# cure-lab/MagicDrive

Measured on AMD Instinct MI355X. Metric: 6-view scenes/sec at 224x400, 50-step DDIM, higher is better.
Workload: dtype bf16; 1 GPU; configs[1]: 6-view 224x400, text-only conditioning (camera_param=None -> CFG off), 50-step DDIM, bf16; scenes_per_gpu=64, ddim_steps=50, scheduler=ddim, parallelism=scene-sharded x1, hipgraph=True, streams=2, output_type=latent

## Files before the change

magicdrive_amd/csrc/gemm_route.h:

```cpp
#pragma once
#include <cstddef>
#include <cstdio>

#if defined(__HIPCC__) || defined(__HIP__)
#define MDX_ROUTE_HD __host__ __device__ __forceinline__
#else
#define MDX_ROUTE_HD inline
#endif

namespace mdx_route {

constexpr int R_EINVAL = -1, R_EUNSUPPORTED = -3;
constexpr int XL_SLOTS = 12;

struct RouteIn {
    int M, N, K, batch, splitk, epi;
    bool c_f32, conv;
    int Hi, Wi, Cin, Ho, Wo, kh, kw, sh, sw, ph, pw;
    bool cimajor, up2;
    int upB;
    long lda, ldw, ldc, ldr, sC;
    int rows_per_b, col_split;
    long ws_bytes;
    bool has_ws, bias, temb, R, Vt, Wq, ln_csum, ln_scratch, ln_stats, rowstat;
    int ln_stats_parts, rowstat_parts;
    bool ln;
    bool wide;
    bool r_al16, wq_al16, bias_al16;
};

struct RouteOpts {
    int GEMM_WS, GEMM_XL, XL_K320, XL_MIN_TILES, XL_BN, XL_GEGLU320, GEMM_SMALL_TILES, GEMM_BM256, GEMM_BM, GEMM_BN, GEMM_BK, GEMM_FLATTEN,
        LN_FUSE, LN_STATS, GEMM_TIMING;
};

enum Main { MAIN_WS, MAIN_XL, MAIN_GENERIC };

struct Route {
    int err;
    const char* msg;
    int arg;
    Main main;
    int bn;
    int BM, BN, BK, splitk, kchunk;
    bool normalise_first;
    bool rowstat_after;
    bool keep_rowstat, keep_ln, keep_ln_stats;
    bool timing;
};

struct UpAxis { int cnt, first, pad, par; };
MDX_ROUTE_HD UpAxis up_axis(int c, int n_in, int n_out) {
    const int crop = n_out != 2 * n_in;
    UpAxis a;
    a.cnt = c == 2 ? 1 : n_in - crop;
    a.first = c == 2 ? n_in - 1 : 0;
    a.pad = c == 1 ? 0 : 1;
    a.par = c == 1 ? 1 : 0;
    return a;
}
MDX_ROUTE_HD int up_mtiles(int upB, int Hi, int Wi, int Ho, int Wo) {
    const int ny = 2 + (Ho != 2 * Hi), nx = 2 + (Wo != 2 * Wi);
    int mt = 0;
    for (int yc = 0; yc < ny; ++yc)
        for (int xc = 0; xc < nx; ++xc) mt += (int)(((long)upB * up_axis(yc, Hi, Ho).cnt * up_axis(xc, Wi, Wo).cnt + 255) / 256);
    return mt;
}

inline bool xl_supported(const RouteIn& p, int bn) {
    const bool conv = p.conv;
    if (p.batch > 1 || p.splitk > 1 || p.c_f32 || (p.N % 4) || (p.K % 64) || p.Vt) return false;
    if (p.col_split && (conv || p.bias || p.temb || p.R || p.epi || (p.sC & 1) || (p.ldc & 1) || p.col_split < 16)) return false;
    if (bn != 256 && bn != 160 && bn != 320) return false;
    if (p.epi == 1 && (bn != 256 || (p.N % 64))) return false;
    if (p.epi == 2) return false;
    if (conv && p.up2) {
        if (bn == 160 || p.kh != 2 || p.kw != 2 || (p.Cin % 64) || p.R || p.temb || p.epi || p.col_split) return false;
        if (p.upB < 1 || p.Hi < 1 || p.Wi < 1 || (p.Ho != 2 * p.Hi && p.Ho != 2 * p.Hi - 1) || (p.Wo != 2 * p.Wi && p.Wo != 2 * p.Wi - 1)) return false;
        if ((long)p.Hi * p.Wi + 256 >= (1L << 24) || (long)p.upB * p.Hi * p.Wi >= 0x7fffff00L) return false;
        const long span = ((long)(256 / p.Wi + 3) * p.Wi + 256L + 2 * p.Wi) * p.lda * 2;
        if (span >= 0x40000000L) return false;
        if ((p.Ho != 2 * p.Hi || p.Wo != 2 * p.Wi) && ((long)p.upB * p.Hi * p.Wi + p.Wi + 2) * p.lda * 2 >= 0x7fff0000L) return false;
    } else if (conv) {
        if (p.kh != 3 || p.kw != 3 || p.ph != 1 || p.pw != 1 || (p.Cin % 64) || !p.cimajor) return false;
        const long span = ((long)(256 / p.Wo + 3) * p.sh * p.Wi + 256L * p.sw + 3 * p.Wi) * p.lda * 2;
        if (span >= 0x40000000L) return false;
    } else if ((long)256 * p.lda * 2 >= 0x40000000L) return false;
    if ((long)bn * p.ldw * 2 >= 0x40000000L) return false;
    if (p.temb && p.epi != 1) {
        const int rows = p.rows_per_b > 0 ? p.rows_per_b : 1;
        if (256 / rows + 2 > XL_SLOTS) return false;
    }
    return true;
}

inline bool ws_supported(const RouteIn& p) {
    return p.K == 320 && p.batch <= 1 && p.splitk <= 1 && !p.c_f32 && !p.temb && (p.epi == 0 || p.epi == 1) && (p.N % 4) == 0 &&
           (p.epi != 1 || (p.N % 64) == 0);
}
inline bool ws_fits_window(const RouteIn& p) { return (long)p.M * p.lda * 2 < 0x7FFF0000L; }
inline bool ws_fuses_layernorm(const RouteIn& p) {
    if (!p.ln_csum || (p.ln_stats && p.ln_stats_parts > 4)) return false;
    return p.epi == 0 || (p.epi == 1 && p.ln_stats);
}
inline bool ws_emits_rowstat(const RouteIn& p) {
    return p.rowstat && p.epi == 0 && !p.Vt && p.wide && !p.c_f32 && !p.ln && (p.N + 127) / 128 <= p.rowstat_parts;
}
inline bool xd_supported(const RouteIn& q) {
    if (!q.Wq || q.batch > 1 || q.splitk > 1 || q.c_f32 || q.Vt || q.col_split || q.temb || q.rowstat || q.ln) return false;
    if (q.epi != 0 && q.epi != 1) return false;
    if (q.epi == 1 && (q.R || (q.N % 64))) return false;
    if ((q.K % 128) || q.K < 640 || (q.N % 16) || !q.wide) return false;
    if (q.R && ((q.ldr % 8) || !q.r_al16)) return false;
    if (!q.wq_al16 || (q.bias && !q.bias_al16)) return false;
    if ((long)256 * q.lda * 2 >= 0x40000000L || (long)256 * q.ldc * 2 >= 0x40000000L || (long)256 * q.ldr * 2 >= 0x40000000L) return false;
    if ((long)16 * (q.K >> 5) * 1024 >= 0x40000000L) return false;
    return true;
}

struct XlWidth { int bn; unsigned bit; double a, b; };
constexpr unsigned W320 = 1, W256 = 2, W160 = 4, W_ALL = 7;
constexpr XlWidth kXlWidths[3] = {{320, W320, 23.7, 1.896}, {256, W256, 13.4, 1.565}, {160, W160, 16.6, 1.116}};
inline unsigned xl_width_bit(int bn) { return bn == 320 ? W320 : bn == 256 ? W256 : bn == 160 ? W160 : 0u; }

inline int xl_pick_width(const RouteIn& p, long mtiles, long min_tiles, unsigned widths) {
    int pick = 0;
    double best = 1e300;
    for (const XlWidth& w : kXlWidths) {
        if (!(widths & w.bit) || !xl_supported(p, w.bn)) continue;
        const long t = mtiles * ((p.N + w.bn - 1) / w.bn);
        if (t < min_tiles) continue;
        const double c = (double)((t + 255) / 256) * (w.a + w.b * (p.K / 64.0));
        if (c < best) { best = c; pick = w.bn; }
    }
    return pick;
}

inline Route route_fail(Route r, int code, const char* msg, int arg = 0) { r.err = code; r.msg = msg; r.arg = arg; return r; }
inline Route route_xl(Route r, int bn) { r.main = MAIN_XL; r.bn = bn; return r; }

inline Route gemm_route_flat(const RouteIn& p, const RouteOpts& o) {
    Route r = {};
    const int bn = o.GEMM_XL > 0 ? xl_pick_width(p, (p.M + 255) / 256, 128, W_ALL) : 0;
    return bn ? route_xl(r, bn) : route_fail(r, R_EUNSUPPORTED, nullptr);
}

inline Route gemm_route(RouteIn p, const RouteOpts& o) {
    Route r = {};
    r.main = MAIN_GENERIC;
    const bool conv = p.conv, geglu = p.epi == 1;
    if (!o.LN_STATS) { p.rowstat = false; p.rowstat_parts = 0; p.ln_stats = false; p.ln_stats_parts = 0; }
    r.keep_rowstat = p.rowstat; r.keep_ln = p.ln; r.keep_ln_stats = p.ln_stats;
    if (p.up2) {
        if (!conv) return route_fail(r, R_EINVAL, "upsample2x: conv only");
        int bn = xl_pick_width(p, up_mtiles(p.upB, p.Hi, p.Wi, p.Ho, p.Wo), 0, W320 | W256);
        if ((o.XL_BN == 320 || o.XL_BN == 256) && xl_supported(p, o.XL_BN)) bn = o.XL_BN;
        if (!bn) return route_fail(r, R_EINVAL, "mdx_conv2d: upsample2x needs Cin %% 64 == 0, Ho in {2 Hi, 2 Hi - 1}, Wo in {2 Wi, 2 Wi - 1}, bias-only epilogue, no split-K; with a cropped axis B * Hi * Wi * ldx * 2 < 2^31");
        return route_xl(r, bn);
    }
    if (geglu && (p.N % 64) != 0) return route_fail(r, R_EINVAL, "GEGLU needs packed N %% 64 == 0 (N=%d)", p.N);
    const long mt256 = (p.M + 255) / 256;
    const bool geglu_xl = o.XL_GEGLU320 && o.GEMM_XL == 1 && !conv && geglu && p.K == 320 && p.splitk <= 1 && o.GEMM_WS < 2 &&
                          xl_supported(p, 256) && mt256 * ((p.N + 255) / 256) >= 1024;
    const bool ws_first = !conv && o.GEMM_WS > 0 && p.splitk <= 1 && ws_supported(p) && ws_fits_window(p) && (o.GEMM_WS >= 2 || p.M >= 8192);
    const bool ws_taken = !geglu_xl && ws_first && !(o.XL_K320 && o.GEMM_XL > 0);
    if (p.rowstat) {
        if (conv || p.batch > 1 || p.epi != 0 || p.c_f32 || p.Vt || p.rowstat_parts < 1) return route_fail(r, R_EINVAL, "rowstat_out: plain 2-D GEMM with 16-bit C only");
        if (!(ws_taken && ws_emits_rowstat(p) && o.LN_FUSE)) {
            r.rowstat_after = true; r.keep_rowstat = false;
            p.rowstat = false; p.rowstat_parts = 0;
        }
    }
    if (p.ln) {
        if (conv || p.batch > 1) return route_fail(r, R_EINVAL, "fused LayerNorm: plain 2-D GEMM only");
        if (!(ws_taken && ws_fuses_layernorm(p) && o.LN_FUSE)) {
            if (!p.ln_scratch) return route_fail(r, R_EINVAL, "fused LayerNorm: this shape is not normalised in-kernel and no ln_scratch was given");
            r.normalise_first = true; r.keep_ln = r.keep_ln_stats = false;
            p.ln = false; p.ln_csum = false; p.ln_stats = false; p.ln_stats_parts = 0;
        }
    }
    const unsigned widths = o.XL_BN ? xl_width_bit(o.XL_BN) : W_ALL;
    if (o.GEMM_XL >= 2 && p.splitk <= 1 && p.batch <= 1 && !(p.K == 320 && !conv && !o.XL_K320)) {
        if (const int bn = xl_pick_width(p, mt256, 0, widths)) return route_xl(r, bn);
    }
    if (geglu_xl) return route_xl(r, 256);
    if (ws_taken) { r.main = MAIN_WS; return r; }
    int BM, BN = 128;
    if (!geglu && (p.N <= 64 || (p.N % 128 != 0 && p.N <= 192))) BN = 64;
    BM = p.M >= 2048 ? 128 : 64;
    if (o.GEMM_SMALL_TILES && p.batch <= 1) {
        const long t64 = (long)((p.M + 63) / 64) * ((p.N + 63) / 64);
        if (geglu) {
            BM = p.M >= 512 ? 128 : 64;
        } else if (!conv) {
            if (t64 <= 1408) BM = BN = 64;
        } else if (t64 * (long)((p.K + 63) / 64) <= 40000) {
            BM = BN = 64;
        } else if (BN == 128) {
            BM = 128;
        }
    }
    if (o.GEMM_BM256 && BN == 128 && p.M >= o.GEMM_BM256) BM = 256;
    if (o.GEMM_BM == 64 || o.GEMM_BM == 128) BM = o.GEMM_BM;
    if ((o.GEMM_BN == 64 && !geglu) || o.GEMM_BN == 128) BN = o.GEMM_BN;
    const long tiles = (long)((p.M + BM - 1) / BM) * ((p.N + BN - 1) / BN) * (p.batch > 1 ? p.batch : 1);
    int splitk = 1;
    if (p.splitk > 0) {
        splitk = p.splitk;
    } else if (p.batch <= 1 && p.has_ws && tiles < 384 && p.K >= 1024 && (p.N % 4) == 0) {
        const long want = (768 + tiles - 1) / tiles;
        const long maxs = p.K / 512;
        splitk = (int)(want < maxs ? (want < 32 ? want : 32) : (maxs < 32 ? maxs : 32));
        if (splitk < 1) splitk = 1;
    }
    if (p.batch > 1) splitk = 1;
    if (splitk > 1) {
        const long per = (long)p.M * p.N * (long)sizeof(float);
        const long fit = per > 0 ? p.ws_bytes / per : 0;
        if (fit < splitk) splitk = fit < 1 ? 1 : (int)fit;
    }
    const int kchunk = ((p.K + splitk - 1) / splitk + 63) / 64 * 64;
    splitk = (p.K + kchunk - 1) / kchunk;
    if (splitk > 1 && !p.has_ws) return route_fail(r, R_EINVAL, "split-K needs a workspace");
    p.splitk = splitk;
    if (splitk == 1 && o.GEMM_XL > 0) {
        if (const int bn = xl_pick_width(p, mt256, o.GEMM_XL >= 2 ? 0 : o.XL_MIN_TILES, widths)) return route_xl(r, bn);
    }
    if (ws_first) { r.main = MAIN_WS; return r; }
    r.BM = BM; r.BN = BN; r.BK = o.GEMM_BK == 32 ? 32 : 64; r.splitk = splitk; r.kchunk = kchunk;
    r.timing = o.GEMM_TIMING && p.has_ws && splitk == 1;
    return r;
}

inline void tag_generic(char* s, size_t n, int BM, int BN, int BK, bool conv) {
    snprintf(s, n, "gemm_conv_kernel<%d,%d,%d,%d,%d,%s>", BM, BN, BK, BM == 256 ? 4 : 2, 2, conv ? "conv" : "gemm");
}
inline void tag_xl(char* s, size_t n, int bn, bool conv, bool up2) {
    snprintf(s, n, "gemm_xl_kernel<256x%d,%s>", bn, conv ? (up2 ? "conv,up2x" : "conv") : "gemm");
}
inline void tag_xlp(char* s, size_t n, bool geglu, bool has_r) {
    snprintf(s, n, "gemm_xlp_kernel<256x256,%s%s>", geglu ? "geglu" : "gemm", has_r ? "+res" : "");
}
inline const char* tag_ws(bool geglu, bool vt, int ln, bool rs) {
    return geglu ? (ln ? "gemm_ws_kernel<geglu,lns>" : "gemm_ws_kernel<geglu>")
                 : ln == 2 ? (vt ? "gemm_ws_kernel<vT,lns>" : "gemm_ws_kernel<plain,lns>")
                 : ln == 1 ? (vt ? "gemm_ws_kernel<vT,ln>" : "gemm_ws_kernel<plain,ln>")
                           : (vt ? "gemm_ws_kernel<vT>" : rs ? "gemm_ws_kernel<plain,rs>" : "gemm_ws_kernel<plain>");
}
inline void route_tag(const Route& r, const RouteIn& p, char* s, size_t n) {
    if (r.main == MAIN_XL) tag_xl(s, n, r.bn, p.conv, p.up2);
    else if (r.main == MAIN_GENERIC) tag_generic(s, n, r.BM, r.BN, r.BK, p.conv);
    else snprintf(s, n, "%s", tag_ws(p.epi == 1, false, !r.keep_ln ? 0 : r.keep_ln_stats ? 2 : 1, r.keep_rowstat));
}

}
```

magicdrive_amd/csrc/gemm_ws.hip:

```cpp
#include "common.h"
#include "launch.h"
#include "options.h"
#include "gemm_params.h"

namespace mdx {

constexpr unsigned WS_OOB = 0xFFFFFF00u;
constexpr unsigned WS_RECORDS = 0x80000000u;

template <int N>
__device__ __forceinline__ void ws_wait_vmcnt() { asm volatile("s_waitcnt vmcnt(%0)" ::"n"(N) : "memory"); }
typedef __attribute__((ext_vector_type(4))) unsigned ws_rsrc_t;
__device__ __forceinline__ void ws_glds(const ws_rsrc_t rs, unsigned lds_addr, unsigned voff) {
    unsigned keep;
    lds_addr = __builtin_amdgcn_readfirstlane(lds_addr);
    asm volatile(
        "s_mov_b32 %0, m0\n\t"
        "s_mov_b32 m0, %1\n\t"
        "s_nop 0\n\t"
        "buffer_load_dwordx4 %2, %3, 0 offen lds\n\t"
        "s_mov_b32 m0, %0"
        : "=&s"(keep)
        : "s"(lds_addr), "v"(voff), "s"(rs)
        : "memory");
}
__device__ __forceinline__ void ws_lds_barrier() {
    asm volatile("s_waitcnt lgkmcnt(0)" ::: "memory");
    __builtin_amdgcn_s_barrier();
    asm volatile("" ::: "memory");
}

template <bool GEGLU, int ST, bool VT, int LN, bool RS>
__global__ __launch_bounds__(256, 2) void gemm_ws_kernel(GCParams p) {
    static_assert(!(GEGLU && LN == 1), "in-kernel LayerNorm statistics: plain and V^T epilogues only");
    static_assert(!(RS && (GEGLU || VT)), "row statistics: plain store phase only");

    constexpr int BM = 128, BN = 128, BK = 64, KS = 20, NSLAB = 5;
    constexpr int BNO = GEGLU ? BN / 2 : BN;
    constexpr int CSTR = BNO + 8;
    constexpr int ROWS_PASS = GEGLU ? 128 : 64;
    constexpr int CSTR_T = ROWS_PASS + 8;
    constexpr int STAGE = BM * BK * 2;
    constexpr int PPW = 4;
    extern __shared__ __attribute__((aligned(16))) unsigned char smem[];
    bf16_t* Cs = (bf16_t*)(smem + ST * STAGE);
    float2* Ls = (float2*)(smem + ST * STAGE + 128 * (64 + 8) * 2);
    float* Lc = (float*)(Ls + 128);
    float* Lb = Lc + 128;

    const int tid = threadIdx.x, lane = tid & 63;
    const int wave = __builtin_amdgcn_readfirstlane(tid >> 6);
    const int frow = lane & 31, half = lane >> 5;
    const int xcd = blockIdx.x & 7, kq = blockIdx.x >> 3;
    const int tn = kq % p.nt;
    const int walker = (kq / p.nt) * 8 + xcd;
    const int nwalk = p.swz;
    const int n0 = tn * BN;
    const int mt = p.mt;
    const int ntiles = walker < mt ? (mt - walker + nwalk - 1) / nwalk : 0;
    if (ntiles == 0) return;

    int wrow, ocol;
    if (GEGLU) {
        const int grp = wave >> 1, hv = wave & 1;
        wrow = n0 + grp * 64 + (frow < 16 ? 16 * hv + frow : 32 + 16 * hv + (frow - 16));
        ocol = grp * 32 + 16 * hv;
    } else {
        wrow = n0 + 32 * wave + frow;
        ocol = 32 * wave;
    }
    Frag8 wf[KS];
    {
        const bf16_t* wp = p.W + (long)min(wrow, p.N - 1) * p.ldw + half * 8;
        const unsigned keep = wrow < p.N ? 0xffffffffu : 0u;
#pragma unroll
        for (int ks = 0; ks < KS; ++ks) wf[ks].u = *(const uint4*)(wp + ks * 16);
#pragma unroll
        for (int ks = 0; ks < KS; ++ks) { wf[ks].u.x &= keep; wf[ks].u.y &= keep; wf[ks].u.z &= keep; wf[ks].u.w &= keep; }
    }
    float4 bA[4];
#pragma unroll
    for (int g = 0; g < 4; ++g) {
        if (LN) { bA[g] = make_float4(0.f, 0.f, 0.f, 0.f); continue; }
        int col;
        if (GEGLU) col = n0 + (wave >> 1) * 64 + 16 * (wave & 1) + 8 * (g & 1) + 4 * half + 32 * (g >> 1);
        else col = n0 + ocol + 8 * g + 4 * half;
        const float4 bv = p.bias ? *(const float4*)(p.bias + min(col, p.N - 4)) : make_float4(0.f, 0.f, 0.f, 0.f);
        bA[g] = col < p.N ? bv : make_float4(0.f, 0.f, 0.f, 0.f);
    }
    float bch = 0.f, csch = 0.f;
    if (VT) {
        bch = p.bias ? p.bias[min(wrow, p.N - 1)] : 0.f;
        if (LN) csch = p.ln_csum[min(wrow, p.N - 1)];
        if (wrow >= p.N) { bch = 0.f; csch = 0.f; }
    }
    if (LN && !VT) {
        if (tid < 128) {
            Lc[tid] = n0 + tid < p.N ? p.ln_csum[n0 + tid] : 0.f;
            Lb[tid] = (p.bias && n0 + tid < p.N) ? p.bias[n0 + tid] : 0.f;
        }
    }

    ws_rsrc_t rsA;
    {
        const unsigned long long a_ = (unsigned long long)p.A;
        rsA.x = __builtin_amdgcn_readfirstlane((unsigned)a_);
        rsA.y = __builtin_amdgcn_readfirstlane((unsigned)(a_ >> 32) & 0xffffu);
        rsA.z = WS_RECORDS; rsA.w = 0x00020000u;
    }
    const unsigned lds0 = (unsigned)(unsigned long long)(__attribute__((address_space(3))) void*)smem;
#pragma unroll
    for (int ks = 0; ks < KS; ++ks) asm volatile("" : "+v"(wf[ks].u.x), "+v"(wf[ks].u.y), "+v"(wf[ks].u.z), "+v"(wf[ks].u.w));
#pragma unroll
    for (int g = 0; g < 4; ++g) asm volatile("" : "+v"(bA[g].x), "+v"(bA[g].y), "+v"(bA[g].z), "+v"(bA[g].w));
    if (VT) asm volatile("" : "+v"(bch), "+v"(csch));
    const int crow = lane >> 3, cphys = lane & 7;
    unsigned r_row[PPW], r_coff[PPW];
#pragma unroll
    for (int j = 0; j < PPW; ++j) {
        const int row = (wave * PPW + j) * 8 + crow;
        r_row[j] = row;
        r_coff[j] = (unsigned)(((cphys ^ ((row >> 1) & 7)) * 8) * 2);
    }
    const unsigned ldab = (unsigned)(p.lda * 2);
    int f_tile = walker, f_slab = 0, f_cnt = 0;
    const int total = ntiles * NSLAB;
#define WS_ISSUE_PIECE(j)                                                                                                       \
    {                                                                                                                           \
        const unsigned m = (unsigned)(f_tile * BM) + r_row[j];                                                                  \
        const unsigned off = (f_cnt < total && m < (unsigned)p.M) ? m * ldab + (unsigned)(f_slab * BK * 2) + r_coff[j] : WS_OOB; \
        ws_glds(rsA, lds0 + (unsigned)((f_cnt % ST) * STAGE + (wave * PPW + (j)) * 1024), off);                                 \
    }
#define WS_ADVANCE()                                                                                                            \
    {                                                                                                                           \
        ++f_cnt;                                                                                                                \
        if (++f_slab == NSLAB) { f_slab = 0; f_tile += nwalk; }                                                                 \
    }

    f32x16_t acc[4];
#pragma unroll
    for (int i = 0; i < 4; ++i)
#pragma unroll
        for (int r = 0; r < 16; ++r) acc[i][r] = 0.f;

#pragma unroll
    for (int s = 0; s < ST - 1; ++s) {
#pragma unroll
        for (int j = 0; j < PPW; ++j) WS_ISSUE_PIECE(j)
        WS_ADVANCE()
    }

    const int x0 = half ^ ((frow >> 1) & 7);
    const unsigned char* const a_rd = smem + frow * 128;
    const bf16_t* Rg = p.R ? (const bf16_t*)p.R : nullptr;
    bf16_t* Cg = (bf16_t*)p.C;
    constexpr bool vtile = VT;
    const int n0o = GEGLU ? n0 / 2 : n0, Nout = GEGLU ? p.N / 2 : p.N;
    int q = 0;
    float s1a = 0.f, s1b = 0.f, s2a = 0.f, s2b = 0.f;
    const float ln_eps = p.ln_eps;
    constexpr int LNS_MAXP = 4;
    unsigned long long lns[LNS_MAXP] = {0, 0, 0, 0};
    for (int t = 0; t < ntiles; ++t) {
        const int m0 = (walker + t * nwalk) * BM;
#pragma unroll
        for (int s = 0; s < NSLAB; ++s, ++q) {
            __builtin_amdgcn_sched_barrier(0);
            ws_wait_vmcnt<(ST - 2) * PPW>();
            if constexpr (LN == 2) {
                if (s == 1) {
#pragma unroll
                    for (int k = 0; k < LNS_MAXP; ++k) asm volatile("" : "+v"(lns[k]));
                    float t1 = 0.f, t2 = 0.f;
#pragma unroll
                    for (int k = 0; k < LNS_MAXP; ++k) {
                        const float keep = k < p.ln_stats_parts ? 1.f : 0.f;
                        t1 = __builtin_fmaf(__uint_as_float((unsigned)(lns[k] & 0xffffffffull)), keep, t1);
                        t2 = __builtin_fmaf(__uint_as_float((unsigned)(lns[k] >> 32)), keep, t2);
                    }
                    const float mean = t1 * (1.0f / 320.0f);
                    const float var = fmaxf(__builtin_fmaf(-mean, mean, t2 * (1.0f / 320.0f)), 0.f);
                    const float rs = rsqrtf(var + ln_eps);
                    if (tid < 128) Ls[tid] = make_float2(rs, -mean * rs);
                }
            }
            __builtin_amdgcn_s_barrier();
            asm volatile("" ::: "memory");
            __builtin_amdgcn_sched_barrier(0);
            if constexpr (LN == 2) {
                if (s == 0) {
                    const long row = min(m0 + (tid & 127), p.M - 1);
#pragma unroll
                    for (int k = 0; k < LNS_MAXP; ++k) {
                        const float* sp = p.ln_stats + ((long)min(k, p.ln_stats_parts - 1) * p.M + row) * 2;
                        asm volatile("global_load_dwordx2 %0, %1, off" : "=v"(lns[k]) : "v"(sp) : "memory");
                    }
                }
            }
#pragma unroll
            for (int j = 0; j < PPW; ++j) WS_ISSUE_PIECE(j)
            WS_ADVANCE()
            const unsigned char* as = a_rd + (q % ST) * STAGE;
            Frag8 af[2][4];
            Frag8 sf[2];
            const unsigned char* sr = as + wave * (32 * 128);
            if constexpr (LN == 1) sf[0].u = *(const uint4*)(sr + (x0 << 4));
#pragma unroll
            for (int i = 0; i < 4; ++i) af[0][i].u = *(const uint4*)(as + i * 32 * 128 + (x0 << 4));
            if constexpr (LN == 1) __builtin_amdgcn_sched_barrier(0); else __builtin_amdgcn_sched_group_barrier(0x100, 4, 0);
#pragma unroll
            for (int ks = 0; ks < 4; ++ks) {
                if (ks + 1 < 4) {
                    const int co = (x0 ^ ((ks + 1) << 1)) << 4;
                    if constexpr (LN == 1) sf[(ks + 1) & 1].u = *(const uint4*)(sr + co);
#pragma unroll
                    for (int i = 0; i < 4; ++i) af[(ks + 1) & 1][i].u = *(const uint4*)(as + i * 32 * 128 + co);
                }
                if constexpr (LN == 1) {
                    if (ks + 1 < 4) __builtin_amdgcn_sched_barrier(0);
#pragma unroll
                    for (int i = 0; i < 4; ++i) {
                        if (vtile) acc[i] = MDX_MFMA_32x32x16(af[ks & 1][i].v, wf[s * 4 + ks].v, acc[i]);
                        else acc[i] = MDX_MFMA_32x32x16(wf[s * 4 + ks].v, af[ks & 1][i].v, acc[i]);
                        const float xa = bf2f(sf[ks & 1].h[2 * i]), xb = bf2f(sf[ks & 1].h[2 * i + 1]);
                        s1a += xa; s1b += xb;
                        s2a = __builtin_fmaf(xa, xa, s2a); s2b = __builtin_fmaf(xb, xb, s2b);
                        asm volatile("" : "+v"(s1a), "+v"(s1b), "+v"(s2a), "+v"(s2b));
                        __builtin_amdgcn_sched_barrier(0);
                    }
                    continue;
                }
                if (vtile) {
#pragma unroll
                    for (int i = 0; i < 4; ++i)
                        acc[i] = MDX_MFMA_32x32x16(af[ks & 1][i].v, wf[s * 4 + ks].v, acc[i]);
                } else {
#pragma unroll
                    for (int i = 0; i < 4; ++i)
                        acc[i] = MDX_MFMA_32x32x16(wf[s * 4 + ks].v, af[ks & 1][i].v, acc[i]);
                }
                if (ks + 1 < 4) __builtin_amdgcn_sched_group_barrier(0x100, 4, 0);
                __builtin_amdgcn_sched_group_barrier(0x008, 4, 0);
            }
            if constexpr (LN == 1) asm volatile("" : "+v"(s1a), "+v"(s1b), "+v"(s2a), "+v"(s2b));
        }
        if constexpr (LN == 1) {
            float s1 = s1a + s1b, s2 = s2a + s2b;
            s1 += __shfl_xor(s1, 32, 64); s2 += __shfl_xor(s2, 32, 64);
            const float mean = s1 * (1.0f / 320.0f);
            const float var = fmaxf(__builtin_fmaf(-mean, mean, s2 * (1.0f / 320.0f)), 0.f);
            const float rs = rsqrtf(var + ln_eps);
            if (half == 0) Ls[wave * 32 + frow] = make_float2(rs, -mean * rs);
            s1a = s1b = s2a = s2b = 0.f;
            ws_lds_barrier();
        }
#pragma unroll
        for (int pass = 0; pass < BM / ROWS_PASS; ++pass) {
            if (pass > 0) ws_lds_barrier();
            if constexpr (VT) {
#pragma unroll
                for (int i = 0; i < 4; ++i) {
                    if (i * 32 / ROWS_PASS != pass) continue;
#pragma unroll
                    for (int g = 0; g < 4; ++g) {
                        const int tl = i * 32 + 8 * g + 4 * half - pass * ROWS_PASS;
                        float o[4];
                        if constexpr (LN != 0) {
                            const float4 sa = *(const float4*)(Ls + i * 32 + 8 * g + 4 * half), sb = *(const float4*)(Ls + i * 32 + 8 * g + 4 * half + 2);
                            o[0] = __builtin_fmaf(sa.x, acc[i][4 * g], __builtin_fmaf(sa.y, csch, bch));
                            o[1] = __builtin_fmaf(sa.z, acc[i][4 * g + 1], __builtin_fmaf(sa.w, csch, bch));
                            o[2] = __builtin_fmaf(sb.x, acc[i][4 * g + 2], __builtin_fmaf(sb.y, csch, bch));
                            o[3] = __builtin_fmaf(sb.z, acc[i][4 * g + 3], __builtin_fmaf(sb.w, csch, bch));
                        } else {
#pragma unroll
                            for (int e = 0; e < 4; ++e) o[e] = acc[i][4 * g + e] + bch;
                        }
                        uint2 ov;
                        ov.x = pack2bf(o[0], o[1]);
                        ov.y = pack2bf(o[2], o[3]);
                        *(uint2*)(Cs + (32 * wave + frow) * CSTR_T + tl) = ov;
                    }
#pragma unroll
                    for (int r = 0; r < 16; ++r) acc[i][r] = 0.f;
                }
                ws_lds_barrier();
                const int mp = m0 + pass * ROWS_PASS;
                constexpr int CPRT = ROWS_PASS / 8;
#pragma unroll
                for (int u = 0; u < 128 * CPRT / 256; ++u) {
                    const int idx = tid + u * 256;
                    const int ch = idx / CPRT, c8 = (idx - ch * CPRT) * 8;
                    const int m = mp + c8, cv = n0 + ch;
                    if (m >= p.M || cv >= p.N) continue;
                    const int b = m / p.vt_T, t = m - b * p.vt_T;
                    *(uint4*)(p.Vt + (long)b * p.vt_stride + (long)cv * p.vt_ld + t) = *(const uint4*)(Cs + ch * CSTR_T + c8);
                }
                continue;
            }
#pragma unroll
            for (int i = 0; i < 4; ++i) {
                if (i * 32 / ROWS_PASS != pass) continue;
                const int ml = i * 32 + frow - pass * ROWS_PASS;
                if (GEGLU) {
#pragma unroll
                    for (int g = 0; g < 2; ++g) {
                        float bvv[4] = {bA[g].x, bA[g].y, bA[g].z, bA[g].w};
                        float bgg[4] = {bA[2 + g].x, bA[2 + g].y, bA[2 + g].z, bA[2 + g].w};
                        float o[4];
                        float cvv[4] = {0.f, 0.f, 0.f, 0.f}, cgg[4] = {0.f, 0.f, 0.f, 0.f};
                        float2 st = make_float2(1.f, 0.f);
                        if constexpr (LN != 0) {
                            st = Ls[i * 32 + frow];
                            const int cb = (wave >> 1) * 64 + 16 * (wave & 1) + 8 * g + 4 * half;
                            const float4 c_v = *(const float4*)(Lc + cb), c_g = *(const float4*)(Lc + cb + 32);
                            const float4 b_v = *(const float4*)(Lb + cb), b_g = *(const float4*)(Lb + cb + 32);
                            cvv[0] = c_v.x; cvv[1] = c_v.y; cvv[2] = c_v.z; cvv[3] = c_v.w;
                            cgg[0] = c_g.x; cgg[1] = c_g.y; cgg[2] = c_g.z; cgg[3] = c_g.w;
                            bvv[0] = b_v.x; bvv[1] = b_v.y; bvv[2] = b_v.z; bvv[3] = b_v.w;
                            bgg[0] = b_g.x; bgg[1] = b_g.y; bgg[2] = b_g.z; bgg[3] = b_g.w;
                        }
#pragma unroll
                        for (int e = 0; e < 4; e += 2) {
                            float x0, x1;
                            f32x2_t gt;
                            if constexpr (LN != 0) {
                                x0 = __builtin_fmaf(st.x, acc[i][4 * g + e], __builtin_fmaf(st.y, cvv[e], bvv[e]));
                                x1 = __builtin_fmaf(st.x, acc[i][4 * g + e + 1], __builtin_fmaf(st.y, cvv[e + 1], bvv[e + 1]));
                                gt.x = __builtin_fmaf(st.x, acc[i][8 + 4 * g + e], __builtin_fmaf(st.y, cgg[e], bgg[e]));
                                gt.y = __builtin_fmaf(st.x, acc[i][8 + 4 * g + e + 1], __builtin_fmaf(st.y, cgg[e + 1], bgg[e + 1]));
                            } else {
                                x0 = acc[i][4 * g + e] + bvv[e]; x1 = acc[i][4 * g + e + 1] + bvv[e + 1];
                                gt.x = acc[i][8 + 4 * g + e] + bgg[e]; gt.y = acc[i][8 + 4 * g + e + 1] + bgg[e + 1];
                            }
                            const f32x2_t ge = gelu_erf_f2(gt);
                            o[e] = x0 * ge.x; o[e + 1] = x1 * ge.y;
                        }
                        uint2 ov; ov.x = pack2bf(o[0], o[1]); ov.y = pack2bf(o[2], o[3]);
                        *(uint2*)(Cs + ml * CSTR + ocol + 8 * g + 4 * half) = ov;
                    }
                } else {
#pragma unroll
                    for (int g = 0; g < 4; ++g) {
                        uint2 ov;
                        if constexpr (LN != 0) {
                            const float2 st = Ls[i * 32 + frow];
                            const float4 cs = *(const float4*)(Lc + ocol + 8 * g + 4 * half), bb = *(const float4*)(Lb + ocol + 8 * g + 4 * half);
                            ov.x = pack2bf(__builtin_fmaf(st.x, acc[i][4 * g], __builtin_fmaf(st.y, cs.x, bb.x)),
                                           __builtin_fmaf(st.x, acc[i][4 * g + 1], __builtin_fmaf(st.y, cs.y, bb.y)));
                            ov.y = pack2bf(__builtin_fmaf(st.x, acc[i][4 * g + 2], __builtin_fmaf(st.y, cs.z, bb.z)),
                                           __builtin_fmaf(st.x, acc[i][4 * g + 3], __builtin_fmaf(st.y, cs.w, bb.w)));
                        } else {
                        ov.x = pack2bf(acc[i][4 * g] + bA[g].x, acc[i][4 * g + 1] + bA[g].y);
                        ov.y = pack2bf(acc[i][4 * g + 2] + bA[g].z, acc[i][4 * g + 3] + bA[g].w);
                        }
                        *(uint2*)(Cs + ml * CSTR + ocol + 8 * g + 4 * half) = ov;
                    }
                }
#pragma unroll
                for (int r = 0; r < 16; ++r) acc[i][r] = 0.f;
            }
            ws_lds_barrier();
            const int mp = m0 + pass * ROWS_PASS;
            if (p.wide) {
                constexpr int CPR = BNO / 8, IT = ROWS_PASS * CPR / 256;
                static_assert(IT == 4, "row walk batch");
                uint4 rv[IT];
                bool ok[IT];
#pragma unroll
                for (int u = 0; u < IT; ++u) {
                    const int idx = tid + u * 256;
                    const int row = idx / CPR, c8 = (idx - row * CPR) * 8;
                    ok[u] = mp + row < p.M && n0o + c8 < Nout;
                }
                if (Rg) {
#pragma unroll
                    for (int u = 0; u < IT; ++u) {
                        const int idx = tid + u * 256;
                        const int row = idx / CPR, c8 = (idx - row * CPR) * 8;
                        const int rr = min(mp + row, p.M - 1), cc = min(n0o + c8, Nout - 8);
                        rv[u] = *(const uint4*)(Rg + (long)rr * p.ldr + cc);
                    }
                }
#pragma unroll
                for (int u = 0; u < IT; ++u) {
                    if (!RS && !ok[u]) continue;
                    const int idx = tid + u * 256;
                    const int row = idx / CPR, c8 = (idx - row * CPR) * 8;
                    uint4 v = *(const uint4*)(Cs + row * CSTR + c8);
                    if (Rg) { v.x = add2bf(v.x, rv[u].x); v.y = add2bf(v.y, rv[u].y); v.z = add2bf(v.z, rv[u].z); v.w = add2bf(v.w, rv[u].w); }
                    if (ok[u]) *(uint4*)(Cg + (long)(mp + row) * p.ldc + n0o + c8) = v;
                    if constexpr (RS) {
                        static_assert(CPR == 16, "row statistics: one 16-lane DPP row per stored row segment");
                        const unsigned km = ok[u] ? 0xffffffffu : 0u;
                        const unsigned one2 = MDX_ONE16 | (MDX_ONE16 << 16);
                        const unsigned w0 = v.x & km, w1 = v.y & km, w2 = v.z & km, w3 = v.w & km;
                        float q1 = dot2_16(w0, one2, 0.f), q2 = dot2_16(w0, w0, 0.f);
                        q1 = dot2_16(w1, one2, q1); q2 = dot2_16(w1, w1, q2);
                        q1 = dot2_16(w2, one2, q1); q2 = dot2_16(w2, w2, q2);
                        q1 = dot2_16(w3, one2, q1); q2 = dot2_16(w3, w3, q2);
#define WS_ROR_ADD(x, n) x += __builtin_bit_cast(float, __builtin_amdgcn_update_dpp(0, __builtin_bit_cast(int, x), 0x120 + (n), 0xf, 0xf, true))
                        WS_ROR_ADD(q1, 8); WS_ROR_ADD(q2, 8); WS_ROR_ADD(q1, 4); WS_ROR_ADD(q2, 4);
                        WS_ROR_ADD(q1, 2); WS_ROR_ADD(q2, 2); WS_ROR_ADD(q1, 1); WS_ROR_ADD(q2, 1);
#undef WS_ROR_ADD
                        if ((tid & 15) == 0 && mp + row < p.M) *(float2*)(p.rowstat + ((long)tn * p.M + mp + row) * 2) = make_float2(q1, q2);
                    }
                }
            } else {
                constexpr int CPR = BNO / 4, IT = ROWS_PASS * CPR / 256;
#pragma unroll 1
                for (int i0 = 0; i0 < IT; i0 += 4) {
                    uint2 rv[4];
                    bool ok[4];
#pragma unroll
                    for (int u = 0; u < 4; ++u) {
                        const int idx = tid + (i0 + u) * 256;
                        const int row = idx / CPR, c4 = (idx - row * CPR) * 4;
                        ok[u] = mp + row < p.M && n0o + c4 < Nout;
                        rv[u] = make_uint2(0, 0);
                        if (Rg && ok[u]) rv[u] = *(const uint2*)(Rg + (long)(mp + row) * p.ldr + n0o + c4);
                    }
#pragma unroll
                    for (int u = 0; u < 4; ++u) {
                        if (!ok[u]) continue;
                        const int idx = tid + (i0 + u) * 256;
                        const int row = idx / CPR, c4 = (idx - row * CPR) * 4;
                        uint2 v = *(const uint2*)(Cs + row * CSTR + c4);
                        if (Rg) { v.x = add2bf(v.x, rv[u].x); v.y = add2bf(v.y, rv[u].y); }
                        *(uint2*)(Cg + (long)(mp + row) * p.ldc + n0o + c4) = v;
                    }
                }
            }
        }
    }
#undef WS_ISSUE_PIECE
#undef WS_ADVANCE
    ws_wait_vmcnt<0>();
}

template <bool GEGLU, bool VT, int LN, bool RS>
static int launch_ws_one(const GCParams& p, hipStream_t st) {
    constexpr int ST = 3;
    const size_t smem = (size_t)ST * 128 * 64 * 2 + (size_t)128 * (64 + 8) * 2 +
                        (LN ? 128 * sizeof(float2) + 256 * sizeof(float) : 0);
    auto kern = gemm_ws_kernel<GEGLU, ST, VT, LN, RS>;
    if (int rc = ensure_dyn_smem((const void*)kern, smem, "ws")) return rc;
    GCParams q = p;
    q.mt = (p.M + 127) / 128; q.nt = (p.N + 127) / 128;
    const int slots = (int)opt(OPT_WS_SLOTS);
    int nwalk = slots / q.nt / 8 * 8;
    if (nwalk < 8) nwalk = 8;
    const int mt8 = (q.mt + 7) / 8 * 8;
    if (nwalk > mt8) nwalk = mt8;
    q.swz = nwalk;
    hipLaunchKernelGGL(kern, dim3((unsigned)(nwalk * q.nt)), dim3(256), smem, st, q);
    return check_launch(mdx_route::tag_ws(GEGLU, VT, LN, RS));
}

static bool ws_fits_window(const GCParams& p) { return mdx_route::ws_fits_window(route_in(p, false)); }
static bool ws_fuses_layernorm(const GCParams& p) { return mdx_route::ws_fuses_layernorm(route_in(p, false)); }
static bool ws_emits_rowstat(const GCParams& p) { return mdx_route::ws_emits_rowstat(route_in(p, false)); }

int launch_gemm_ws(const GCParams& p, hipStream_t st) {
    if (!ws_fits_window(p)) return set_error(MDX_EINVAL, "gemm_ws: A exceeds the 2 GiB buffer window (M * lda * 2 = %ld bytes; the transposed-V output has no other main loop)", (long)p.M * p.lda * 2);
    const bool ln = p.ln_eps > 0.f;
    if (ln && !ws_fuses_layernorm(p)) return set_error(MDX_EINVAL, "gemm_ws: fused LayerNorm needs ln_csum and a plain epilogue (GEGLU: also ln_stats)");
    const bool lns = ln && p.ln_stats != nullptr;
    if (p.rowstat) {
        if (!ws_emits_rowstat(p)) return set_error(MDX_EINVAL, "gemm_ws: rowstat_out needs the plain wide store phase and one part per 128-column tile");
        const int ntile = (p.N + 127) / 128;
        if (p.rowstat_parts > ntile)
            if (hipMemsetAsync(p.rowstat + (long)ntile * p.M * 2, 0, (size_t)(p.rowstat_parts - ntile) * p.M * 2 * sizeof(float), st) != hipSuccess)
                return set_error(MDX_ELAUNCH, "gemm_ws: rowstat memset");
        return launch_ws_one<false, false, 0, true>(p, st);
    }
    if (p.epi == 1) return lns ? launch_ws_one<true, false, 2, false>(p, st) : launch_ws_one<true, false, 0, false>(p, st);
    auto plain = [&](const GCParams& c) {
        return lns ? launch_ws_one<false, false, 2, false>(c, st) : ln ? launch_ws_one<false, false, 1, false>(c, st) : launch_ws_one<false, false, 0, false>(c, st);
    };
    if (!p.Vt) return plain(p);
    GCParams c = p;
    c.N = p.vt_from; c.Vt = nullptr;
    int rc = plain(c);
    if (rc != MDX_OK) return rc;
    GCParams v = p;
    v.W = p.W + (long)p.vt_from * p.ldw; v.N = p.N - p.vt_from; v.bias = p.bias ? p.bias + p.vt_from : nullptr; v.R = nullptr; v.C = nullptr;
    v.ln_csum = p.ln_csum ? p.ln_csum + p.vt_from : nullptr;
    return lns ? launch_ws_one<false, true, 2, false>(v, st) : ln ? launch_ws_one<false, true, 1, false>(v, st) : launch_ws_one<false, true, 0, false>(v, st);
}

}
```

magicdrive_amd/csrc/options.h:

```cpp
#pragma once
#include <cstdint>

namespace mdx_rt {
int64_t opt(int id);
}

namespace mdx {

#define MDX_OPTIONS(X) \
    X(ATTN_SWZ, 2, "XCD-aware block order of attention.hip: 0 off, 1 per (view, head), 2 per view (all heads of a view on one XCD)") \
    X(ATTN_NW4_BLOCKS, 256L, "attention.hip: 4-wave workgroups from this many blocks") \
    X(ATTN_NW8_BLOCKS, (1L << 40), "attention.hip: 8-wave workgroups from this many blocks") \
    X(ATTN_NW, 0, "force the waves per workgroup of attention.hip (0 = heuristic)") \
    X(ATTN2, 1, "attention2.hip for head dim 40") \
    X(ATTN3, 0, "only in `make ATTN3=1` builds: tools/attn3/attention3.hip (permute-free P, QK of the next kv tile beside this tile's softmax) for the head-dim-40 FOLD launches: self, cross-view, joint") \
    X(ATTN3_WGS, 0, "attention3.hip: persistent workgroups per XCD (0 = automatic: two per CU)") \
    X(ATTN2_PF, 1, "attention2.hip, head dim 40 FOLD 32-query form: permute-free P (PV on 32x32x16 MFMAs, K rows permuted so that a lane's scores are its PV operand)") \
    X(ATTN2_D80, 2, "attention2.hip for head dim 80: 0 never, 1 always, 2 only the two-source cross-view form") \
    X(ATTN2_FOLD, 1, "attention2.hip: subtract the running maximum inside the QK MFMA when Q is pre-scaled (head dim 40)") \
    X(ATTN2_RES, 1, "attention2.hip: kv sequences of <= 3 tiles (text context) resident in LDS, one workgroup per (view, head) walks the query blocks: 0 off, 1 for launches of >= 1024 (view, head) pairs, 2 whenever supported") \
    X(ATTN2_VIEWMAP, 1, "attention2.hip block order: 1 = all heads and query blocks of a view on one XCD (a row's 128-byte lines are shared by the heads), 0 = per (view, head)") \
    X(ATTN2_QT, 0, "32-query tiles per wave in attention2.hip: 0 = automatic (2; 1 for one-source FOLD launches), 1 / 2 = force") \
    X(CONV_OUT_WS, 1, "direct conv with Cout <= 4 and a long K (conv_out): weight-stationary K-parallel kernel (weights in registers, 16 pixels per wave)") \
    X(GEMM_SWZ, 1, "XCD-aware tile order of the generic kernel") \
    X(GEMM_SMALL_TILES, 1, "generic tile choice for small grids (1-4 scenes per call): 64 x 64 for plain GEMMs up to 1408 such tiles and for convs up to 40 k (tile, slab) units, 128 x 128 for larger convs with M < 2048, 128-row GEGLU from M = 512; 0 = the rounds 1-5 rule (128 rows from M = 2048, else 64 x 128)") \
    X(GEMM_BM, 0, "force the generic tile's rows (64 / 128; 0 = heuristic)") \
    X(GEMM_BN, 0, "force the generic tile's columns (64 / 128; 0 = heuristic)") \
    X(GEMM_PIPE, 1, "software-pipelined fragment reads in the generic 128x128x64 tile") \
    X(EPI_WIDE, 1, "16-byte epilogue accesses when alignment allows") \
    X(GEMM_WS, 1, "gemm_ws.hip: 0 off, 1 when M >= 8192, 2 whenever supported") \
    X(GEMM_XL, 1, "gemm_xl.hip: 0 off, 1 cost model, 2 whenever supported") \
    X(XL_K320, 0, "let XL take the K = 320 projections from gemm_ws.hip") \
    X(XL_MIN_TILES, 64, "fewest 256-row tiles an XL launch must have (round 6: 64; 160 until then — 2...8 scenes per call are 2-6 % faster with the lower bound, 12+ scenes and 1 scene do not care: profiles/r06_lat1_small_grids.log)") \
    X(XL_BN, 0, "force an XL tile width (160 / 256 / 320; 0 = cost model)") \
    X(XL_GEGLU320, 0, "K = 320 GEGLU on the 256-wide XL tile instead of gemm_ws.hip") \
    X(GEMM_BM256, 0, "generic 256x128 8-wave tile from M >= value (0 = never)") \
    X(GEMM_TIMING, 0, "s_memtime stamps of the generic kernel into the op workspace") \
    X(GEMM_BK, 64, "generic tile slab depth (64 or 32)") \
    X(GEMM_FLATTEN, 1, "batched shared-A GEMM as ONE col_split XL launch") \
    X(CONV_CIMAJOR, 1, "channel-block-major K order of implicit-GEMM convs") \
    X(WS_SLOTS, 512, "workgroup slots the gemm_ws M walkers are sized for") \
    X(XL_TIMING, 0, "per-workgroup s_memtime stamps into the op workspace") \
    X(GN_REVERSE, 1, "two-stage GroupNorm: statistics pass reads the tensor back to front (Infinity-Cache reuse between producer / passes)") \
    X(GN_FINALIZE_CHUNKS, 16, "two-stage GroupNorm: with more chunks per image than this the chunk partials are combined once by gn_finalize_kernel (0 = always in the apply pass)") \
    X(GN_ONE_KERNEL_ELEMS, (4L << 20), "GroupNorm tensors of at most this many elements (all images) take the one-launch kernel (one workgroup per (image, group)) instead of the two streaming passes") \
    X(GN_TWO_STAGE, 1, "streaming two-stage GroupNorm for maps >= 32768 elements") \
    X(XL_PERSIST, 1, "256x256 XL GEMMs (plain / GEGLU, optional residual) on the persistent kernel gemm_xlp_kernel") \
    X(XD, 0, "W-direct persistent GEMM (gemm_xd.hip: weights global -> registers, finished tile stored under the next tile's main loop) for the 256x256 XL GEMMs whose descriptor carries Wq (K % 128 == 0, K >= 640); bit-identical to gemm_xlp_kernel, measured 0.89-1.04x of it (profiles/r06_xd_ab.log): off by default") \
    X(XL_RASTER, 2, "XL tile order: 0 row-major, 1 XCD-strided M-tiles, 2 XCD-blocked (M-group x N-group panels per XCD)") \
    X(XL_GM, 0, "XL_RASTER 2: force the M-tiles per panel (0 = cost model, xl_layout.h: raster_shape)") \
    X(XL_GN, 0, "XL_RASTER 2: force the N-tiles per panel (0 = cost model)") \
    X(STREAMS, 2, "host side (pipeline): HIP streams a pipe() call spreads its scene chunks over (chunks of >= 16 scenes, one plan + hipGraph each)") \
    X(PLAN_CACHE, 6, "host side (pipeline): sampler plans (captured graphs + buffers) kept per pipeline (LRU); a multi-stream call pins one plan per chunk") \
    X(CHECK_TIMESTEPS, 0, "host side (schedulers): 1 = a device-resident timestep that is not in the scheduler's list raises (one sync per step) instead of poisoning the sample with NaN") \
    X(LN_FUSE, 1, "MdxGemmDesc.ln_eps: 1 = gemm_ws.hip normalises the rows in-kernel, 0 = always normalise into ln_scratch first (A/B)") \
    X(LN_STATS, 1, "MdxGemmDesc.rowstat_out / ln_stats: 1 = row statistics travel from the producer's store phase to the fused LayerNorm, 0 = round-5 behaviour (nothing emitted, in-kernel sums, GEGLU through ln_scratch) (A/B)")

enum Opt : int {
#define MDX_OPT_ENUM(key, dflt, doc) OPT_##key,
    MDX_OPTIONS(MDX_OPT_ENUM)
#undef MDX_OPT_ENUM
    OPT_COUNT
};

using mdx_rt::opt;

}
```

Baseline: 7.586 scenes/s.

## Add 8-wave 128x256 tile variant to gemm_ws for GEGLU with folded LayerNorm

Templates the weight-stationary GEMM kernel on wave count so that an 8-wave workgroup covers 256 output columns. Each activation slab fetched into LDS then feeds twice as many columns, which halves activation traffic per output. By default the wide tile is taken only for the GEGLU epilogue with precomputed LayerNorm stats when N>=512 and M>=8192. The trade is one workgroup per CU instead of two, deeper staging (5 stages), and more LDS, which may reduce latency hiding.

```diff
diff --git a/magicdrive_amd/csrc/gemm_route.h b/magicdrive_amd/csrc/gemm_route.h
--- a/magicdrive_amd/csrc/gemm_route.h
+++ b/magicdrive_amd/csrc/gemm_route.h
@@ -253,4 +253,11 @@
     else snprintf(s, n, "%s", tag_ws(p.epi == 1, false, !r.keep_ln ? 0 : r.keep_ln_stats ? 2 : 1, r.keep_rowstat));
 }
 
-}
+enum WsKind { WS_PLAIN = 0, WS_GEGLU = 1, WS_VT = 2, WS_RS = 3, WS_GEGLU_LNS = 4 };
+inline int ws_tile_cols(int N, int M, int kind, int ws_wide) {
+    if (ws_wide <= 0 || (kind != WS_PLAIN && kind != WS_GEGLU && kind != WS_GEGLU_LNS) || N <= 128) return 128;
+    if (ws_wide >= 2) return 256;
+    return kind == WS_GEGLU_LNS && N >= 512 && M >= 8192 ? 256 : 128;
+}
+
+}
diff --git a/magicdrive_amd/csrc/gemm_ws.hip b/magicdrive_amd/csrc/gemm_ws.hip
--- a/magicdrive_amd/csrc/gemm_ws.hip
+++ b/magicdrive_amd/csrc/gemm_ws.hip
@@ -30,23 +30,23 @@
     asm volatile("" ::: "memory");
 }
 
-template <bool GEGLU, int ST, bool VT, int LN, bool RS>
-__global__ __launch_bounds__(256, 2) void gemm_ws_kernel(GCParams p) {
+template <bool GEGLU, int ST, bool VT, int LN, bool RS, int NW>
+__global__ __launch_bounds__(64 * NW, NW == 4 ? 2 : 1) void gemm_ws_kernel(GCParams p) {
     static_assert(!(GEGLU && LN == 1), "in-kernel LayerNorm statistics: plain and V^T epilogues only");
     static_assert(!(RS && (GEGLU || VT)), "row statistics: plain store phase only");
-
+    constexpr int TN = 32 * NW, NT = 64 * NW; static_assert(NW == 4 || (NW == 8 && !VT && !RS), "256-column tile: plain / GEGLU"); static_assert(ST >= 3 && ST <= 5, "LN == 2 publishes the row statistics before the barrier of slab ST - 2 <= NSLAB - 2");
     constexpr int BM = 128, BN = 128, BK = 64, KS = 20, NSLAB = 5;
-    constexpr int BNO = GEGLU ? BN / 2 : BN;
+    constexpr int BNO = GEGLU ? TN / 2 : TN;
     constexpr int CSTR = BNO + 8;
     constexpr int ROWS_PASS = GEGLU ? 128 : 64;
     constexpr int CSTR_T = ROWS_PASS + 8;
     constexpr int STAGE = BM * BK * 2;
-    constexpr int PPW = 4;
+    constexpr int PPW = 16 / NW, CS_BYTES = NW == 4 ? BN * (64 + 8) * 2 : 128 * (128 + 8) * 2; static_assert(ROWS_PASS * CSTR * 2 <= CS_BYTES && (!VT || 128 * CSTR_T * 2 <= CS_BYTES), "staging");
     extern __shared__ __attribute__((aligned(16))) unsigned char smem[];
     bf16_t* Cs = (bf16_t*)(smem + ST * STAGE);
-    float2* Ls = (float2*)(smem + ST * STAGE + 128 * (64 + 8) * 2);
+    float2* Ls = (float2*)(smem + ST * STAGE + CS_BYTES);
     float* Lc = (float*)(Ls + 128);
-    float* Lb = Lc + 128;
+    float* Lb = Lc + TN;
 
     const int tid = threadIdx.x, lane = tid & 63;
     const int wave = __builtin_amdgcn_readfirstlane(tid >> 6);
@@ -55,7 +55,7 @@
     const int tn = kq % p.nt;
     const int walker = (kq / p.nt) * 8 + xcd;
     const int nwalk = p.swz;
-    const int n0 = tn * BN;
+    const int n0 = tn * TN;
     const int mt = p.mt;
     const int ntiles = walker < mt ? (mt - walker + nwalk - 1) / nwalk : 0;
     if (ntiles == 0) return;
@@ -95,7 +95,7 @@
         if (wrow >= p.N) { bch = 0.f; csch = 0.f; }
     }
     if (LN && !VT) {
-        if (tid < 128) {
+        if (tid < TN) {
             Lc[tid] = n0 + tid < p.N ? p.ln_csum[n0 + tid] : 0.f;
             Lb[tid] = (p.bias && n0 + tid < p.N) ? p.bias[n0 + tid] : 0.f;
         }
@@ -168,7 +168,7 @@
             __builtin_amdgcn_sched_barrier(0);
             ws_wait_vmcnt<(ST - 2) * PPW>();
             if constexpr (LN == 2) {
-                if (s == 1) {
+                if (s == ST - 2) {
 #pragma unroll
                     for (int k = 0; k < LNS_MAXP; ++k) asm volatile("" : "+v"(lns[k]));
                     float t1 = 0.f, t2 = 0.f;
@@ -203,8 +203,9 @@
             const unsigned char* as = a_rd + (q % ST) * STAGE;
             Frag8 af[2][4];
             Frag8 sf[2];
-            const unsigned char* sr = as + wave * (32 * 128);
-            if constexpr (LN == 1) sf[0].u = *(const uint4*)(sr + (x0 << 4));
+            const unsigned char* sr = as + (wave & 3) * (32 * 128);
+            const bool sums = NW == 4 || wave < 4;
+            if constexpr (LN == 1) { if (sums) sf[0].u = *(const uint4*)(sr + (x0 << 4)); }
 #pragma unroll
             for (int i = 0; i < 4; ++i) af[0][i].u = *(const uint4*)(as + i * 32 * 128 + (x0 << 4));
             if constexpr (LN == 1) __builtin_amdgcn_sched_barrier(0); else __builtin_amdgcn_sched_group_barrier(0x100, 4, 0);
@@ -212,7 +213,7 @@
             for (int ks = 0; ks < 4; ++ks) {
                 if (ks + 1 < 4) {
                     const int co = (x0 ^ ((ks + 1) << 1)) << 4;
-                    if constexpr (LN == 1) sf[(ks + 1) & 1].u = *(const uint4*)(sr + co);
+                    if constexpr (LN == 1) { if (sums) sf[(ks + 1) & 1].u = *(const uint4*)(sr + co); }
 #pragma unroll
                     for (int i = 0; i < 4; ++i) af[(ks + 1) & 1][i].u = *(const uint4*)(as + i * 32 * 128 + co);
                 }
@@ -222,9 +223,11 @@
                     for (int i = 0; i < 4; ++i) {
                         if (vtile) acc[i] = MDX_MFMA_32x32x16(af[ks & 1][i].v, wf[s * 4 + ks].v, acc[i]);
                         else acc[i] = MDX_MFMA_32x32x16(wf[s * 4 + ks].v, af[ks & 1][i].v, acc[i]);
-                        const float xa = bf2f(sf[ks & 1].h[2 * i]), xb = bf2f(sf[ks & 1].h[2 * i + 1]);
-                        s1a += xa; s1b += xb;
-                        s2a = __builtin_fmaf(xa, xa, s2a); s2b = __builtin_fmaf(xb, xb, s2b);
+                        if (sums) {
+                            const float xa = bf2f(sf[ks & 1].h[2 * i]), xb = bf2f(sf[ks & 1].h[2 * i + 1]);
+                            s1a += xa; s1b += xb;
+                            s2a = __builtin_fmaf(xa, xa, s2a); s2b = __builtin_fmaf(xb, xb, s2b);
+                        }
                         asm volatile("" : "+v"(s1a), "+v"(s1b), "+v"(s2a), "+v"(s2b));
                         __builtin_amdgcn_sched_barrier(0);
                     }
@@ -250,7 +253,7 @@
             const float mean = s1 * (1.0f / 320.0f);
             const float var = fmaxf(__builtin_fmaf(-mean, mean, s2 * (1.0f / 320.0f)), 0.f);
             const float rs = rsqrtf(var + ln_eps);
-            if (half == 0) Ls[wave * 32 + frow] = make_float2(rs, -mean * rs);
+            if (half == 0 && (NW == 4 || wave < 4)) Ls[(wave & 3) * 32 + frow] = make_float2(rs, -mean * rs);
             s1a = s1b = s2a = s2b = 0.f;
             ws_lds_barrier();
         }
@@ -362,20 +365,20 @@
             ws_lds_barrier();
             const int mp = m0 + pass * ROWS_PASS;
             if (p.wide) {
-                constexpr int CPR = BNO / 8, IT = ROWS_PASS * CPR / 256;
+                constexpr int CPR = BNO / 8, IT = ROWS_PASS * CPR / NT;
                 static_assert(IT == 4, "row walk batch");
                 uint4 rv[IT];
                 bool ok[IT];
 #pragma unroll
                 for (int u = 0; u < IT; ++u) {
-                    const int idx = tid + u * 256;
+                    const int idx = tid + u * NT;
                     const int row = idx / CPR, c8 = (idx - row * CPR) * 8;
                     ok[u] = mp + row < p.M && n0o + c8 < Nout;
                 }
                 if (Rg) {
 #pragma unroll
                     for (int u = 0; u < IT; ++u) {
-                        const int idx = tid + u * 256;
+                        const int idx = tid + u * NT;
                         const int row = idx / CPR, c8 = (idx - row * CPR) * 8;
                         const int rr = min(mp + row, p.M - 1), cc = min(n0o + c8, Nout - 8);
                         rv[u] = *(const uint4*)(Rg + (long)rr * p.ldr + cc);
@@ -384,13 +387,13 @@
 #pragma unroll
                 for (int u = 0; u < IT; ++u) {
                     if (!RS && !ok[u]) continue;
-                    const int idx = tid + u * 256;
+                    const int idx = tid + u * NT;
                     const int row = idx / CPR, c8 = (idx - row * CPR) * 8;
                     uint4 v = *(const uint4*)(Cs + row * CSTR + c8);
                     if (Rg) { v.x = add2bf(v.x, rv[u].x); v.y = add2bf(v.y, rv[u].y); v.z = add2bf(v.z, rv[u].z); v.w = add2bf(v.w, rv[u].w); }
                     if (ok[u]) *(uint4*)(Cg + (long)(mp + row) * p.ldc + n0o + c8) = v;
                     if constexpr (RS) {
-                        static_assert(CPR == 16, "row statistics: one 16-lane DPP row per stored row segment");
+                        static_assert(CPR == 16 && NW == 4, "row statistics: one 16-lane DPP row per stored row segment");
                         const unsigned km = ok[u] ? 0xffffffffu : 0u;
                         const unsigned one2 = MDX_ONE16 | (MDX_ONE16 << 16);
                         const unsigned w0 = v.x & km, w1 = v.y & km, w2 = v.z & km, w3 = v.w & km;
@@ -406,14 +409,14 @@
                     }
                 }
             } else {
-                constexpr int CPR = BNO / 4, IT = ROWS_PASS * CPR / 256;
+                constexpr int CPR = BNO / 4, IT = ROWS_PASS * CPR / NT;
 #pragma unroll 1
                 for (int i0 = 0; i0 < IT; i0 += 4) {
                     uint2 rv[4];
                     bool ok[4];
 #pragma unroll
                     for (int u = 0; u < 4; ++u) {
-                        const int idx = tid + (i0 + u) * 256;
+                        const int idx = tid + (i0 + u) * NT;
                         const int row = idx / CPR, c4 = (idx - row * CPR) * 4;
                         ok[u] = mp + row < p.M && n0o + c4 < Nout;
                         rv[u] = make_uint2(0, 0);
@@ -422,7 +425,7 @@
 #pragma unroll
                     for (int u = 0; u < 4; ++u) {
                         if (!ok[u]) continue;
-                        const int idx = tid + (i0 + u) * 256;
+                        const int idx = tid + (i0 + u) * NT;
                         const int row = idx / CPR, c4 = (idx - row * CPR) * 4;
                         uint2 v = *(const uint2*)(Cs + row * CSTR + c4);
                         if (Rg) { v.x = add2bf(v.x, rv[u].x); v.y = add2bf(v.y, rv[u].y); }
@@ -437,23 +440,33 @@
     ws_wait_vmcnt<0>();
 }
 
-template <bool GEGLU, bool VT, int LN, bool RS>
+#ifndef WS_WIDE_ST
+#define WS_WIDE_ST 5
+#endif
+template <bool GEGLU, bool VT, int LN, bool RS, int NW>
 static int launch_ws_one(const GCParams& p, hipStream_t st) {
-    constexpr int ST = 3;
-    const size_t smem = (size_t)ST * 128 * 64 * 2 + (size_t)128 * (64 + 8) * 2 +
-                        (LN ? 128 * sizeof(float2) + 256 * sizeof(float) : 0);
-    auto kern = gemm_ws_kernel<GEGLU, ST, VT, LN, RS>;
-    if (int rc = ensure_dyn_smem((const void*)kern, smem, "ws")) return rc;
+    constexpr int ST = NW == 4 ? 3 : WS_WIDE_ST, BN = 32 * NW;
+    const size_t smem = (size_t)ST * 128 * 64 * 2 +
+                        (NW == 4 ? (size_t)128 * (64 + 8) * 2 : (size_t)128 * (128 + 8) * 2) +
+                        (LN ? 128 * sizeof(float2) + 2 * BN * sizeof(float) : 0);
+    auto kern = gemm_ws_kernel<GEGLU, ST, VT, LN, RS, NW>;
+    if (int rc = ensure_dyn_smem((const void*)kern, smem, NW == 4 ? "ws" : "ws 256-column")) return rc;
     GCParams q = p;
-    q.mt = (p.M + 127) / 128; q.nt = (p.N + 127) / 128;
-    const int slots = (int)opt(OPT_WS_SLOTS);
+    q.mt = (p.M + 127) / 128; q.nt = (p.N + BN - 1) / BN;
+    const int slots = (int)opt(OPT_WS_SLOTS) * 4 / NW;
     int nwalk = slots / q.nt / 8 * 8;
     if (nwalk < 8) nwalk = 8;
     const int mt8 = (q.mt + 7) / 8 * 8;
     if (nwalk > mt8) nwalk = mt8;
     q.swz = nwalk;
-    hipLaunchKernelGGL(kern, dim3((unsigned)(nwalk * q.nt)), dim3(256), smem, st, q);
+    hipLaunchKernelGGL(kern, dim3((unsigned)(nwalk * q.nt)), dim3(64 * NW), smem, st, q);
     return check_launch(mdx_route::tag_ws(GEGLU, VT, LN, RS));
+}
+template <bool GEGLU, int LN>
+static int launch_ws_cols(const GCParams& p, hipStream_t st) {
+    const int kind = GEGLU ? (LN == 2 ? mdx_route::WS_GEGLU_LNS : mdx_route::WS_GEGLU) : mdx_route::WS_PLAIN;
+    if (mdx_route::ws_tile_cols(p.N, p.M, kind, (int)opt(OPT_WS_WIDE)) == 256) return launch_ws_one<GEGLU, false, LN, false, 8>(p, st);
+    return launch_ws_one<GEGLU, false, LN, false, 4>(p, st);
 }
 
 static bool ws_fits_window(const GCParams& p) { return mdx_route::ws_fits_window(route_in(p, false)); }
@@ -471,11 +484,11 @@
         if (p.rowstat_parts > ntile)
             if (hipMemsetAsync(p.rowstat + (long)ntile * p.M * 2, 0, (size_t)(p.rowstat_parts - ntile) * p.M * 2 * sizeof(float), st) != hipSuccess)
                 return set_error(MDX_ELAUNCH, "gemm_ws: rowstat memset");
-        return launch_ws_one<false, false, 0, true>(p, st);
-    }
-    if (p.epi == 1) return lns ? launch_ws_one<true, false, 2, false>(p, st) : launch_ws_one<true, false, 0, false>(p, st);
+        return launch_ws_one<false, false, 0, true, 4>(p, st);
+    }
+    if (p.epi == 1) return lns ? launch_ws_cols<true, 2>(p, st) : launch_ws_cols<true, 0>(p, st);
     auto plain = [&](const GCParams& c) {
-        return lns ? launch_ws_one<false, false, 2, false>(c, st) : ln ? launch_ws_one<false, false, 1, false>(c, st) : launch_ws_one<false, false, 0, false>(c, st);
+        return lns ? launch_ws_cols<false, 2>(c, st) : ln ? launch_ws_cols<false, 1>(c, st) : launch_ws_cols<false, 0>(c, st);
     };
     if (!p.Vt) return plain(p);
     GCParams c = p;
@@ -485,7 +498,7 @@
     GCParams v = p;
     v.W = p.W + (long)p.vt_from * p.ldw; v.N = p.N - p.vt_from; v.bias = p.bias ? p.bias + p.vt_from : nullptr; v.R = nullptr; v.C = nullptr;
     v.ln_csum = p.ln_csum ? p.ln_csum + p.vt_from : nullptr;
-    return lns ? launch_ws_one<false, true, 2, false>(v, st) : ln ? launch_ws_one<false, true, 1, false>(v, st) : launch_ws_one<false, true, 0, false>(v, st);
-}
-
-}
+    return lns ? launch_ws_one<false, true, 2, false, 4>(v, st) : ln ? launch_ws_one<false, true, 1, false, 4>(v, st) : launch_ws_one<false, true, 0, false, 4>(v, st);
+}
+
+}
diff --git a/magicdrive_amd/csrc/options.h b/magicdrive_amd/csrc/options.h
--- a/magicdrive_amd/csrc/options.h
+++ b/magicdrive_amd/csrc/options.h
@@ -40,6 +40,7 @@
     X(GEMM_FLATTEN, 1, "batched shared-A GEMM as ONE col_split XL launch") \
     X(CONV_CIMAJOR, 1, "channel-block-major K order of implicit-GEMM convs") \
     X(WS_SLOTS, 512, "workgroup slots the gemm_ws M walkers are sized for") \
+    X(WS_WIDE, 1, "gemm_ws.hip: 128 x 256 tiles (8 waves, one workgroup per CU, the activation slab fetched once per 256 columns) for the plain and GEGLU epilogues: 0 never, 1 by the measured rule of ws_tile_cols (gemm_route.h: the GEGLU with folded LayerNorm), 2 whenever N > 128; same bits as the 128-column form") \
     X(XL_TIMING, 0, "per-workgroup s_memtime stamps into the op workspace") \
     X(GN_REVERSE, 1, "two-stage GroupNorm: statistics pass reads the tensor back to front (Infinity-Cache reuse between producer / passes)") \
     X(GN_FINALIZE_CHUNKS, 16, "two-stage GroupNorm: with more chunks per image than this the chunk partials are combined once by gn_finalize_kernel (0 = always in the apply pass)") \
```

New measurement: 7.588 scenes/s, median of 3. About the same (+0.0%).
